# tsirigos/ibm-cbc-genomic-tools

Hardware: AMD Instinct MI355X
Metric: overlap-counted reads/sec, 100M reads x 1M ref intervals (higher is better)
Workload: dtype int32; 1 GPU; BASELINE config 3: 100000000 50bp reads in total, sorted by (chrom,start), x 1000000 ref intervals over 24 hg38 chromosomes, strand ignored (genomic_overlaps count -S -i); reads resident in HBM; total_reads=100000000, refs=1000000, reduce=none (one rank)

## Files before the change

### ibm-cbc-genomic-tools_amd/csrc/gtx_capi.hip

```cpp
#include <hip/hip_runtime.h>
#include <stdint.h>
#include <string.h>
#include <stdio.h>
#include <algorithm>
#include <functional>
#include <string>
#include <thread>
#include <vector>
#include "gtx.h"
#include "gtx_kernels.h"
#include "gtx_pairs.h"
#include "gtx_join.h"
#include "gtx_offset.h"
#include "gtx_signal.h"
#include "gtx_text.h"
#include "gtx_internal.h"

typedef unsigned long long u64;

static thread_local std::string g_create_error;

namespace {

template <class T, bool Pinned> class Buf {
 public:
  size_t cap = 0;
  Buf() = default;
  Buf(Buf &&o) noexcept { *this = std::move(o); }
  Buf &operator=(Buf &&o) noexcept { if (this != &o) { reset(); std::swap(cap, o.cap); std::swap(p_, o.p_); } return *this; }
  ~Buf() { reset(); }
  T *get() const { return p_; }
  explicit operator bool() const { return p_ != nullptr; }
  void reset() { if (p_) (void)(Pinned ? hipHostFree(p_) : hipFree(p_)); p_ = nullptr; cap = 0; }
  hipError_t alloc(size_t n)
  {
    reset();
    const hipError_t e = Pinned ? hipHostMalloc((void **)&p_, sizeof(T) * n) : hipMalloc((void **)&p_, sizeof(T) * n);
    if (e == hipSuccess) cap = n;
    return e;
  }
  hipError_t reserve(size_t need, size_t room) { if (need <= cap) return hipSuccess; hipError_t e = alloc(room); if (e == hipSuccess) cap = need; return e; }
  hipError_t reserve(size_t n) { return reserve(n, n); }
  hipError_t grow(size_t n) { return reserve(std::max<size_t>(n, 1)); }
 private:
  T *p_ = nullptr;
};
template <class T> using DevBuf = Buf<T, false>;
template <class T> using PinBuf = Buf<T, true>;

struct PlaceTable {
  DevBuf<int4> cls; DevBuf<int> rank; int shift = 0;
  gtx::PlaceTable view() const { gtx::PlaceTable t; t.cls = cls.get(); t.rank = rank.get(); t.shift = shift; return t; }
};

struct BucketTables {
  DevBuf<int> bkt; DevBuf<int4> clsCell; DevBuf<uint16_t> cellTab; int nB = 0, nCells = 0, cellShift = 0;
  gtx::BucketTable view() const
  {
    gtx::BucketTable t;
    const int *d = bkt.get();
    t.posHi = d; t.eLo = d + nB; t.eHi = d + 2 * nB; t.sLo = d + 3 * nB; t.sHi = d + 4 * nB; t.cls = d + 5 * nB; t.clsStart = d + 6 * nB; t.nB = nB;
    t.clsCell = clsCell.get(); t.cellTab = cellTab.get(); t.nCells = nCells; t.cellShift = cellShift;
    return t;
  }
};

struct BucketCuts { std::vector<int32_t> posHi, eLo, eHi, sLo, sHi, cls, clsStart; };

struct HistSet { DevBuf<u64> histA, histB, partA, partB, prefA, prefB; DevBuf<unsigned> flags; unsigned epoch = 0; unsigned long long draws = 0; };

struct CountIndex {
  DevBuf<int> sortedE, sortedS, segStart, posE, posS, classBase;
  DevBuf<int> sampE, sampS; int sampShift = 6, nSamp = 0;
  DevBuf<int> topE, topS;
  PlaceTable place;
  BucketTables bkt;
  HistSet hist;
  HistSet alt[GTXI_SHARE_STREAMS];
  DevBuf<gtx::DevInfo> info3; unsigned shareSeq = 0; unsigned shareTurn[GTXI_SHARE_STREAMS] = {}; const gtx::DevInfo *lastShareInfo = nullptr;
};

struct CoverIndex {
  DevBuf<u64> cov[12];
  DevBuf<int> sortedT, segT, topT, posTE, posTS, classBaseT;
  int64_t histLenT = 0;
  PlaceTable place;
  BucketTables bkt;
  bool ready = false;
};

struct RefExtras {
  DevBuf<int> refS, refE, refC;
  int nSpecial = 0; DevBuf<int4> specialRefs; DevBuf<int> specialIdx; DevBuf<u64> specialOut;
  struct PairIdx { DevBuf<int> mem; int n = 0; bool built = false; gtx::PairIndex ix = {}; } pairMulti, pairAll;
  DevBuf<int2> blkOf, blkIv; bool refBlocks = false;
  DevBuf<u64> pairAcc;
  DevBuf<long long> joinKey; std::vector<long long> h_joinKey; int joinMono = -1;
  DevBuf<int4> offRef; DevBuf<int8_t> refStrand;
  bool sigSet = false; double sigMin = 0, sigMax = 0; int64_t sigBins = 0; DevBuf<long long> sigRefLen;
};

struct Share { bool on = false; DevBuf<int> tiles; int nTiles = 0; DevBuf<int> regions; int64_t nRegions = 0, offset = 0; DevBuf<unsigned char> owned; };

struct TextSlot {
  DevBuf<char> text; DevBuf<unsigned> seg;
  DevBuf<unsigned> nl; DevBuf<int> tri, w;
  DevBuf<int> tri2; DevBuf<unsigned> blk; DevBuf<int> w2;
  DevBuf<int> flag; PinBuf<int> hostFlag; PinBuf<char> pin, seam; DevBuf<unsigned long long> sum;
  hipEvent_t evParsed = nullptr, evConsumed = nullptr, evCopied = nullptr; bool busy = false;
};

}

struct gtx_ctx {
  int device = 0;
  hipStream_t stream = nullptr;
  std::string err;

  int64_t nRefs = -1, nValid = 0;
  int nClasses = 0;
  std::vector<int32_t> h_seg;
  CountIndex ix;
// ... 10 lines not shown
  DevBuf<int4> side; DevBuf<unsigned> sideCount; int sideCap = 1 << 20; bool sideUsed = false;
  int specialMode = 0;
  bool tileSumsValid = true;
  int64_t histLen = 0;
  bool pairUsed = false;
  DevBuf<int4> pairQ; DevBuf<int2> pairQBlk, pairQIv;
  DevBuf<long long> joinOff, joinPart, joinCut; DevBuf<int> joinPairs, joinScratch; DevBuf<unsigned> joinBig;
  DevBuf<int> joinReads; DevBuf<int2> joinQBlk, joinQIv;
  DevBuf<gtx::JoinInfo> joinInfo;
  int64_t joinBuffer = 1ll << 26;
  DevBuf<long long> offInv, offOut, offCnt, offPart; DevBuf<int8_t> offQStrand;
  DevBuf<gtx::SignalInfo> sigInfo; DevBuf<unsigned long long> sigBins; DevBuf<long long> sigW;

  DevBuf<gtx::DevInfo> d_info;
  int infoCur = 0;
  PinBuf<gtx::DevInfo> h_info;

  hipStream_t copyStream = nullptr;
  DevBuf<char> stage[2]; DevBuf<int> stageW[2];
  PinBuf<char> pin[2];
  hipEvent_t evCopied[2] = {nullptr, nullptr}, evConsumed[2] = {nullptr, nullptr}; bool slotBusy[2] = {false, false};
  long long stageSeq = 0; bool directPending = false;
  int copyThreads = 8;
  DevBuf<u64> out;
  DevBuf<char> scratch;
  TextSlot text[2];
  long long textSeq = 0;
  DevBuf<int> textTable; DevBuf<char> textNames; unsigned textMask = 0, textBlobLen = 0;
  std::string textBlob;

  DevBuf<u64> micro;
  DevBuf<long long> scanTab;
  std::vector<long long> scanKey;
  int64_t scanTotalWindows = 0, scanTotalMicro = 0, scanTotalTiles = 0;
  BucketTables bktS; DevBuf<gtx::ScanPart> scanParts; int nScanParts = 0; std::vector<long long> scanBktKey; DevBuf<gtx::DevInfo> scanInfo;
  int64_t scanOwnBlocks = 0; DevBuf<long long> scanBounds; DevBuf<int> scanFlag;
  DevBuf<char> resReads; DevBuf<int> resWeights; hipEvent_t evRes[2] = {nullptr, nullptr};

  static constexpr int kProfSlots = 64;
  bool prof = false; long long profCalls = 0;
  int profEvery = 1; long long profSeq = 0; bool profThis = false;
  hipEvent_t evRing[kProfSlots][4] = {};
  hipEvent_t *ev = evRing[0];

  bool streamOpen = false; int64_t streamSeen = 0; int32_t streamLast[2] = {0, 0};
  struct ScanOpen { bool open = false, weighted = false; gtx::ScanArgs a; std::vector<int32_t> classLen; int64_t extent = 0; char prep = '1'; uint32_t flags = 0;
                    DevBuf<unsigned long long> labelSum; } scan;
  int64_t seamUnsorted = INT64_MAX;

  int64_t batchReads = 8ll << 20;
  int chunksPerWave = 0;
  int64_t waveSlots = 8192;
  int prefetch = 4;
};

#define HIPCHK(ctx, call) do { hipError_t e_ = (call); if (e_ != hipSuccess) { \
    (ctx)->err = std::string(#call) + ": " + hipGetErrorString(e_); return GTX_E_HIP; } } while (0)

static int fail(gtx_ctx *c, int code, const char *msg) { c->err = msg; return code; }

template <class T> static hipError_t upload(DevBuf<T> &b, const T *v, size_t n)
{
  hipError_t e = b.alloc(n);
  return e == hipSuccess ? hipMemcpy(b.get(), v, sizeof(T) * n, hipMemcpyHostToDevice) : e;
}

static int make_hist_set(gtx_ctx *c, HistSet &h, int64_t histLen)
{
  const size_t parts = (size_t)gtx::scan_tiles(histLen) + 2;
  HIPCHK(c, h.histA.alloc(histLen)); HIPCHK(c, h.histB.alloc(histLen)); HIPCHK(c, h.partA.alloc(parts)); HIPCHK(c, h.partB.alloc(parts));
  HIPCHK(c, h.prefA.alloc(histLen)); HIPCHK(c, h.prefB.alloc(histLen)); HIPCHK(c, h.flags.alloc(8 * parts));
  for (DevBuf<u64> *b : {&h.histA, &h.histB, &h.partA, &h.partB}) HIPCHK(c, hipMemset(b->get(), 0, sizeof(u64) * b->cap));
  HIPCHK(c, hipMemset(h.flags.get(), 0, sizeof(unsigned) * h.flags.cap));
  h.epoch = 0; h.draws = 0;
  return GTX_OK;
}

static int make_place_table(gtx_ctx *c, const std::vector<int32_t> &seg, const std::vector<int32_t> &arrA, const std::vector<int32_t> &arrB,
                            int nClasses, int64_t nv, PlaceTable &out)
{
  const int64_t budget = std::max<int64_t>(1024, nv / 8) + 2 * (int64_t)nClasses;
  auto cellsOf = [&](int cl, int sh) -> int64_t {
    if (seg[cl] == seg[cl + 1]) return 0;
    const int64_t top = std::max<int64_t>(0, std::max(arrA[seg[cl + 1] - 1], arrB[seg[cl + 1] - 1]));
    return (top >> sh) + 2;
  };
  int sh = 0;
  for (;; sh++) { int64_t t = 0; for (int cl = 0; cl < nClasses; cl++) t += cellsOf(cl, sh); if (t <= budget || sh >= 31) break; }
  std::vector<int4> pc(std::max(nClasses, 1));
  std::vector<int32_t> rank;
  for (int cl = 0; cl < nClasses; cl++) {
    const int64_t nc = cellsOf(cl, sh);
    pc[cl] = make_int4(seg[cl], seg[cl + 1], (int)(rank.size() / 2), (int)nc);
    int32_t ia = seg[cl], ib = seg[cl];
    for (int64_t k = 0; k < nc; k++) {
      const int64_t first = k << sh;
      if (k > 0) { while (ia < seg[cl + 1] && arrA[ia] < first) ia++; while (ib < seg[cl + 1] && arrB[ib] < first) ib++; }
      rank.push_back(ia); rank.push_back(ib);
    }
  }
  rank.push_back(0); rank.push_back(0);
  out.cls.reset(); out.rank.reset();
  HIPCHK(c, out.cls.alloc(pc.size()));
  HIPCHK(c, out.rank.alloc(rank.size()));
  HIPCHK(c, hipMemcpy(out.cls.get(), pc.data(), sizeof(int4) * pc.size(), hipMemcpyHostToDevice));
  HIPCHK(c, hipMemcpy(out.rank.get(), rank.data(), sizeof(int32_t) * rank.size(), hipMemcpyHostToDevice));
  out.shift = sh;
  return GTX_OK;
}

static int build_bucket_tables(gtx_ctx *c, BucketTables &t, BucketCuts &k, int nClasses, bool sync = false)
{
  t.nB = 0;
  const int nB = (int)k.posHi.size();
  if (nB == 0) return GTX_OK;
  const std::vector<int32_t> &posHi = k.posHi, &clsStart = k.clsStart;
  const int kCells = 4096;
  int sh = 0;
  auto cellsAt = [&](int shift) {
    int64_t total = 0;
    for (int cl = 0; cl < nClasses; cl++) {
      const int b0 = clsStart[cl], b1 = clsStart[cl + 1];
      total += b1 - b0 <= 1 ? b1 - b0 : ((((int64_t)posHi[b1 - 2] - posHi[b0]) >> shift) + 1);
    }
// ... 22 lines not shown
  if (sync) HIPCHK(c, hipStreamSynchronize(c->stream));
  HIPCHK(c, upload(t.bkt, all.data(), all.size()));
  HIPCHK(c, t.clsCell.alloc((size_t)nClasses + 1));
  HIPCHK(c, hipMemcpy(t.clsCell.get(), clsCell.data(), sizeof(int32_t) * clsCell.size(), hipMemcpyHostToDevice));
  HIPCHK(c, upload(t.cellTab, cellTab.data(), cellTab.size()));
  t.nB = nB;
  return GTX_OK;
}

extern "C" {

int gtx_version(void) { return 100; }

gtx_ctx *gtx_create(int device_id)
{
  int n = 0;
  hipError_t e = hipGetDeviceCount(&n);
  if (e != hipSuccess || n <= 0) {
    g_create_error = std::string("gtx_create: no usable HIP device (") + (e != hipSuccess ? hipGetErrorString(e) : "device count 0") +
                     "); this library has no CPU path";
    return nullptr;
  }
  if (device_id < 0 || device_id >= n) { g_create_error = "gtx_create: device id out of range"; return nullptr; }
  if ((e = hipSetDevice(device_id)) != hipSuccess) { g_create_error = std::string("hipSetDevice: ") + hipGetErrorString(e); return nullptr; }
  gtx_ctx *c = new gtx_ctx();
  c->device = device_id;
  { int cus = 0; if (hipDeviceGetAttribute(&cus, hipDeviceAttributeMultiprocessorCount, device_id) == hipSuccess && cus > 0) c->waveSlots = 32ll * cus; }
  if (c->d_info.alloc(2) != hipSuccess || c->h_info.alloc(2) != hipSuccess) {
    g_create_error = "gtx_create: allocation failed"; delete c; return nullptr;
  }
  gtx::DevInfo *hi = c->h_info.get();
  hi[1].first_unsorted = INT64_MAX; hi[1].n_no_class = 0; hi[1].n_degenerate = 0; hi[1].first_degenerate = INT64_MAX; hi[1].n_unplaced = 0; hi[1].fault = 0;
  hi[0] = hi[1];
  if (hipMemcpy(c->d_info.get(), &hi[1], sizeof(gtx::DevInfo), hipMemcpyHostToDevice) != hipSuccess ||
      hipMemcpy(c->d_info.get() + 1, &hi[1], sizeof(gtx::DevInfo), hipMemcpyHostToDevice) != hipSuccess) {
    g_create_error = "gtx_create: hipMemcpy failed"; delete c; return nullptr;
  }
  for (auto &slot : c->evRing) for (auto &ev : slot) if (hipEventCreate(&ev) != hipSuccess) { g_create_error = "gtx_create: hipEventCreate failed"; delete c; return nullptr; }
  if (hipStreamCreateWithFlags(&c->copyStream, hipStreamNonBlocking) != hipSuccess) { g_create_error = "gtx_create: hipStreamCreate failed"; delete c; return nullptr; }
  for (int k = 0; k < 2; k++)
    if (hipEventCreateWithFlags(&c->evCopied[k], hipEventDisableTiming) != hipSuccess || hipEventCreateWithFlags(&c->evConsumed[k], hipEventDisableTiming) != hipSuccess ||
        hipEventCreateWithFlags(&c->evRes[k], hipEventDisableTiming) != hipSuccess) {
      g_create_error = "gtx_create: hipEventCreate failed"; delete c; return nullptr;
    }
  { unsigned hc = std::thread::hardware_concurrency(); c->copyThreads = (int)std::max(1u, std::min(hc ? hc : 4u, 8u));
    if (const char *ct = getenv("GTX_COPY_THREADS")) if (atoi(ct) > 0) c->copyThreads = atoi(ct); }
  const char *cpw = getenv("GTX_CHUNKS_PER_WAVE");
  if (cpw && atoi(cpw) > 0) c->chunksPerWave = atoi(cpw);
  const char *br = getenv("GTX_BATCH_READS");
  if (br && atoll(br) > 0) c->batchReads = atoll(br);
  if (const char *bm = getenv("GTX_BUCKET_MIN_READS")) c->bucketMinReads = atoll(bm);
  const char *pf = getenv("GTX_READS_PER_LANE");
  if (pf && atoi(pf) > 0) c->prefetch = atoi(pf);
  return c;
}

void gtx_destroy(gtx_ctx *c)
{
  if (!c) return;
  (void)hipSetDevice(c->device);
  if (c->copyStream) (void)hipStreamSynchronize(c->copyStream);
  for (int k = 0; k < 2; k++)
    for (hipEvent_t e : {c->evCopied[k], c->evConsumed[k], c->evRes[k]}) if (e) (void)hipEventDestroy(e);
  if (c->copyStream) (void)hipStreamDestroy(c->copyStream);
  for (auto &t : c->text) for (hipEvent_t e : {t.evParsed, t.evConsumed, t.evCopied}) if (e) (void)hipEventDestroy(e);
  for (auto &slot : c->evRing) for (auto &ev : slot) if (ev) (void)hipEventDestroy(ev);
  delete c;
}

const char *gtx_last_error(const gtx_ctx *c) { return c ? c->err.c_str() : g_create_error.c_str(); }

int gtx_set_stream(gtx_ctx *c, void *s) { if (!c) return GTX_E_ARG; c->stream = (hipStream_t)s; return GTX_OK; }

int gtx_sync(gtx_ctx *c)
{
  if (!c) return GTX_E_ARG;
  HIPCHK(c, hipSetDevice(c->device));
  HIPCHK(c, hipStreamSynchronize(c->copyStream));
  HIPCHK(c, hipStreamSynchronize(c->stream));
  return GTX_OK;
}

void *gtx_host_alloc(gtx_ctx *c, size_t bytes)
{
  if (!c) return nullptr;
  void *p = nullptr;
  if (hipSetDevice(c->device) != hipSuccess || hipHostMalloc(&p, bytes ? bytes : 1, hipHostMallocPortable) != hipSuccess) { c->err = "gtx_host_alloc: hipHostMalloc failed"; (void)hipGetLastError(); return nullptr; }
  return p;
}

void gtx_host_free(gtx_ctx *c, void *p) { (void)c; if (p) (void)hipHostFree(p); }

int64_t gtx_n_refs(const gtx_ctx *c) { return c ? c->nRefs : -1; }

int gtx_set_refs(gtx_ctx *c, const int32_t *tri, int64_t m, int32_t nClasses) { return gtx_set_refs_ex(c, tri, m, nClasses, 0); }

int gtx_set_refs_ex(gtx_ctx *c, const int32_t *tri, int64_t m, int32_t nClasses, uint32_t flags)
{
  if (!c || m < 0 || (m > 0 && !tri)) return c ? fail(c, GTX_E_ARG, "gtx_set_refs: bad argument") : GTX_E_ARG;
  if (m >= (int64_t)INT32_MAX - 4096) return fail(c, GTX_E_ARG, "gtx_set_refs: too many reference regions");
  HIPCHK(c, hipSetDevice(c->device));
  int maxc = -1;
  for (int64_t k = 0; k < m; k++) {
    int32_t cl = tri[3 * k], s = tri[3 * k + 1], e = tri[3 * k + 2];
    if (cl < -1) return fail(c, GTX_E_RANGE, "gtx_set_refs: negative class id");
    if (s >= INT32_MAX - 1 || e >= INT32_MAX - 1) return fail(c, GTX_E_RANGE, "gtx_set_refs: coordinate >= 2^31-2");
// ... 227 lines not shown
static int pairs_batch(gtx_ctx *c, const void *d_reads, const void *d_weights, int64_t n)
{
  if (c->rx.pairMulti.n > 0) {
    HIPCHK(c, gtx::launch_pair_miss(d_reads, d_weights, n, c->rx.pairMulti.ix, gtx::RegionBlocks{c->rx.blkOf.get(), c->rx.blkIv.get()}, c->rx.pairAcc.get() + c->nRefs, c->stream));
    c->pairUsed = true;
  }
  return GTX_OK;
}

static int merge_batch(gtx_ctx *c, const void *d_reads, const void *d_weights, int64_t n)
{
  if (c->sideUsed && c->rx.nSpecial) HIPCHK(c, gtx::launch_special_refs(d_reads, d_weights, n, c->rx.specialRefs.get(), c->rx.nSpecial, c->specialMode, c->rx.specialOut.get(), c->stream));
  return GTX_OK;
}

static int merge_end(gtx_ctx *c, void *d_out)
{
  if (c->pairUsed) {
    c->pairUsed = false;
    HIPCHK(c, gtx::launch_pair_apply((u64 *)d_out, c->rx.pairAcc.get(), c->rx.pairAcc.get() + c->nRefs, c->nRefs, c->stream));
  }
  if (!c->sideUsed) return GTX_OK;
  c->sideUsed = false;
  HIPCHK(c, gtx::launch_side_reads(c->rx.refC.get(), c->rx.refS.get(), c->rx.refE.get(), c->nRefs, c->side.get(), c->sideCount.get(), c->sideCap, c->specialMode, (u64 *)d_out,
                                   c->d_info.get() + c->infoCur, c->stream));
  HIPCHK(c, gtx::launch_special_scatter(c->rx.specialIdx.get(), c->rx.specialOut.get(), c->rx.nSpecial, (u64 *)d_out, c->sideCount.get(), c->stream));
  return GTX_OK;
}

static int count_begin(gtx_ctx *c)
{
  if (c->histDirty) {
    HistSet &h = c->ix.hist;
    for (DevBuf<u64> *b : {&h.histA, &h.histB, &h.partA, &h.partB}) HIPCHK(c, hipMemsetAsync(b->get(), 0, sizeof(u64) * b->cap, c->stream));
  }
  if (c->histDirty || c->covDirty) HIPCHK(c, hipMemcpyAsync(c->d_info.get() + c->infoCur, &c->h_info.get()[1], sizeof(gtx::DevInfo), hipMemcpyHostToDevice, c->stream));
  if ((c->histDirty || c->covDirty) && c->sideCount.get()) {
    HIPCHK(c, hipMemsetAsync(c->sideCount.get(), 0, sizeof(unsigned), c->stream));
    if (c->rx.nSpecial) HIPCHK(c, hipMemsetAsync(c->rx.specialOut.get(), 0, sizeof(u64) * c->rx.nSpecial, c->stream));
  }
  if (c->histDirty && c->rx.pairAcc.get()) HIPCHK(c, hipMemsetAsync(c->rx.pairAcc.get(), 0, sizeof(u64) * 2 * (size_t)std::max<int64_t>(c->nRefs, 1), c->stream));
  c->sideUsed = false; c->pairUsed = false;
  c->histDirty = true; c->tileSumsValid = true;
  c->ix.lastShareInfo = nullptr;
  return GTX_OK;
}

static int finalize_set(gtx_ctx *c, HistSet &h, bool sumsValid, u64 *d_hits, gtx::DevInfo *info, gtx::DevInfo *infoNext, hipStream_t s,
                        const gtx::FinalizeShare *fs, bool hist32)
{
  if (++h.epoch == 0) { HIPCHK(c, hipMemsetAsync(h.flags.get(), 0, sizeof(unsigned) * h.flags.cap, s)); h.epoch = 1; h.draws = 0; }
  HIPCHK(c, gtx::launch_finalize(h.histA.get(), h.histB.get(), c->histLen, h.partA.get(), h.partB.get(), sumsValid, h.prefA.get(), h.prefB.get(),
                                 c->ix.posE.get(), c->ix.posS.get(), c->ix.classBase.get(), c->nRefs, d_hits, infoNext, s, fs, h.flags.get(), h.epoch, info,
                                 &h.draws, hist32));
  return GTX_OK;
}

static int count_end(gtx_ctx *c, void *d_hits, bool share = false, bool scatter = false, bool hist32 = false)
{
  const gtx::FinalizeShare fs = {c->share.tiles.get(), c->share.nTiles, c->share.regions.get(), c->share.nRegions, scatter};
  int rc = finalize_set(c, c->ix.hist, c->tileSumsValid, (u64 *)d_hits, c->d_info.get() + c->infoCur, c->d_info.get() + (c->infoCur ^ 1), c->stream,
                        share ? &fs : nullptr, hist32);
  if (rc) return rc;
  rc = merge_end(c, d_hits); if (rc) return rc;
  c->histDirty = false;
  c->infoCur ^= 1;
  return GTX_OK;
}

int gtx_count_device(gtx_ctx *c, const void *d_reads, const void *d_weights, int64_t n, uint32_t flags, void *d_hits)
{
  if (!c) return GTX_E_ARG;
  if (c->nRefs < 0) return fail(c, GTX_E_STATE, "gtx_count_device: gtx_set_refs has not been called");
  if (n < 0 || (n > 0 && !d_reads) || (c->nRefs > 0 && !d_hits)) return fail(c, GTX_E_ARG, "gtx_count_device: bad argument");
  HIPCHK(c, hipSetDevice(c->device));
  int rc = count_begin(c); if (rc) return rc;
  c->profThis = c->prof && (c->profEvery <= 1 || (c->profSeq++ % c->profEvery) == 0);
  if (c->profThis) { c->ev = c->evRing[c->profCalls % gtx_ctx::kProfSlots]; HIPCHK(c, hipEventRecord(c->ev[1], c->stream)); }
  rc = merge_prepare(c, flags, 0); if (rc) return rc;
  const bool streaming = (flags & (GTX_READS_SORTED | GTX_CHECK_SORTED)) != 0;
  if (!streaming) c->tileSumsValid = false;
  bool h32 = false;
  if (streaming) {
    const gtx::CountArgs a = count_args(c, c->ix.hist, flags, n, 0, COUNT_ANY, d_weights == nullptr);
    h32 = a.hist32 != 0 && n > 0;
    HIPCHK(c, gtx::launch_count(d_reads, d_weights, n, a, true, c->stream));
  }
  else { rc = launch_unsorted(c, d_reads, d_weights, n, count_args(c, c->ix.hist, flags, n)); if (rc) return rc; }
  rc = merge_batch(c, d_reads, d_weights, n); if (rc) return rc;
  rc = pairs_batch(c, d_reads, d_weights, n); if (rc) return rc;
  if (c->profThis) HIPCHK(c, hipEventRecord(c->ev[2], c->stream));
  rc = count_end(c, d_hits, false, false, h32); if (rc) return rc;
  if (c->profThis) { if (c->profEvery <= 1) HIPCHK(c, hipEventRecord(c->ev[3], c->stream)); c->profCalls++; }
  return GTX_OK;
}

static void info_out(const gtx::DevInfo &d, gtx_count_info *o, int64_t base)
{
  o->first_unsorted = d.first_unsorted == INT64_MAX ? -1 : d.first_unsorted + base;
  o->n_no_class = d.n_no_class; o->n_degenerate = d.n_degenerate;
  o->first_degenerate = d.first_degenerate == INT64_MAX ? -1 : d.first_degenerate + base;
  o->n_unplaced = d.n_unplaced;
}

static int fault_check(gtx_ctx *c, const gtx::DevInfo &d)
{
  return d.fault ? fail(c, GTX_E_HIP, "the finalize step gave up waiting for a tile sum (finalize_scan_chained_kernel): the result of this call is void; GTX_CHAINED_SCAN=0 takes the two-launch finalize") : GTX_OK;
// ... 1606 lines not shown
```

### ibm-cbc-genomic-tools_amd/csrc/gtx_kernels.h

```cpp
#pragma once
#include <hip/hip_runtime.h>
#include <stdint.h>
#include <mutex>

namespace gtx {

struct PerDevice {
  std::mutex m; unsigned long long done = 0;
  template <class F> hipError_t once(F fn)
  {
    int dev = 0;
    hipError_t e = hipGetDevice(&dev);
    if (e != hipSuccess) return e;
    std::lock_guard<std::mutex> lk(m);
    if (dev >= 0 && dev < 64 && ((done >> dev) & 1)) return hipSuccess;
    e = fn();
    if (e == hipSuccess && dev >= 0 && dev < 64) done |= 1ull << dev;
    return e;
  }
};

struct DevInfo {
  long long first_unsorted;
  long long n_no_class;
// ... 93 lines not shown
  const int *cls;
  const int *clsStart;
  int nB;
  const int4 *clsCell;
  const unsigned short *cellTab;
  int nCells, cellShift;
};
struct BucketWork {
  void *tmpReads; int *tmpWeights;
  unsigned arenaPairs;
  unsigned *dir;
  unsigned *list;
  unsigned *chunkCount;
  unsigned *rowOff;
  unsigned *arenaUsed;
};
struct BucketPlan { int per, line; unsigned blocks; size_t arenaPairs, pairs, chunks, matrix; };
BucketPlan bucket_plan(long long n, int nClasses, int nB, int nCells, bool weighted);
bool bucket_tables_fit(int nClasses, int nB, int nCells);
int bucket_e_size();
int bucket_s_size();
int bucket_t_size();
hipError_t launch_count_bucketed(const void *reads, const void *weights, long long n, const CountArgs &a, const BucketTable &t,
                                 const BucketWork &w, const BucketPlan &p, hipStream_t st);
hipError_t launch_cover_bucketed(const void *reads, const void *weights, long long n, const CountArgs &a, const CoverArgs &cv, const BucketTable &t,
                                 const BucketWork &w, const BucketPlan &p, hipStream_t st);
struct ScanPart { int bucket, first, count, pad; };
int scan_part_bins(bool weighted);
hipError_t launch_scan_bucketed(const void *reads, const void *weights, long long n, const CountArgs &a, const ScanArgs &sc, const BucketTable &t,
                                const BucketWork &w, const BucketPlan &p, const ScanPart *parts, int nParts, hipStream_t st,
                                unsigned long long *out = nullptr);
int scan_fused_max_comb();
hipError_t launch_tile_sums(unsigned long long *histA, unsigned long long *histB, long long histLen, unsigned long long *tileA, unsigned long long *tileB, hipStream_t st);

hipError_t launch_special_refs(const void *reads, const void *weights, long long n, const int4 *refs, int nSpecial, int mode,
                               unsigned long long *out, hipStream_t st);
hipError_t launch_side_reads(const int *refC, const int *refS, const int *refE, long long m, const int4 *side, const unsigned *sideCount,
                             int sideCap, int mode, unsigned long long *hits, DevInfo *info, hipStream_t st);
hipError_t launch_special_scatter(const int *specialIdx, unsigned long long *specialOut, int nSpecial, unsigned long long *hits,
                                  unsigned *sideCount, hipStream_t st);

SpanSchedule span_schedule(long long nChunks, int cpw, int r, long long slots);
int search_sample_shift(long long nValid);
int scan_tiles(long long len);

hipError_t launch_count(const void *reads, const void *weights, long long n, const CountArgs &a, bool sortedHint, hipStream_t st);
struct FinalizeShare { const int *tileList; int nTiles; const int *regionList; long long nRegions; bool scatter; };
hipError_t launch_finalize(unsigned long long *histA, unsigned long long *histB, long long histLen,
                           unsigned long long *tileA, unsigned long long *tileB, bool tileSumsValid,
                           unsigned long long *prefA, unsigned long long *prefB,
                           const int *posE, const int *posS, const int *classBase, long long m,
                           unsigned long long *hits, DevInfo *nextInfo, hipStream_t st, const FinalizeShare *share = nullptr,
                           unsigned *chainFlags = nullptr, unsigned epoch = 0, DevInfo *info = nullptr, unsigned long long *chainDraws = nullptr,
                           bool hist32 = false);
hipError_t launch_coverage(const void *reads, const void *weights, long long n, const CoverArgs &a, hipStream_t st);
hipError_t launch_coverage_finalize(const CoverArgs &a, long long histLen, const CoverGather &g, long long m,
                                    unsigned long long *cov, DevInfo *nextInfo, hipStream_t st);
hipError_t launch_scan_zero(void *micro, long long bytes, const int *runIf, hipStream_t st);
hipError_t launch_scan_hist(const void *reads, const void *weights, long long n, const ScanArgs &a, hipStream_t st, const int *runIf = nullptr);
int scan_window_tile();
hipError_t launch_scan_windows(const void *micro, bool micro64, const ScanArgs &a, long long totalTiles,
                               unsigned long long *out, hipStream_t st, const int *runIf = nullptr);

struct ScanOwn {
  const long long *blkOff;
  int tile;
  long long totalBlocks;
  long long *bounds;
  int *flag;
};
int scan_own_tile(long long nReads, long long totalMicro, int comb);
hipError_t launch_scan_own(const void *reads, const void *weights, long long n, const ScanArgs &a, const ScanOwn &o,
                           unsigned long long *out, hipStream_t st);

}
```

### ibm-cbc-genomic-tools_amd/csrc/gtx_kernels.hip

```cpp
#include <hip/hip_runtime.h>
#include <stdint.h>
#include <stdlib.h>
#include <string.h>
#include <stdio.h>
#include <type_traits>
#include <vector>
#include <algorithm>
#include "gtx_kernels.h"

namespace gtx {

typedef unsigned long long u64;
typedef long long i64;

static constexpr int kHi = 0x7fffffff;
static constexpr int kLo = (int)0x80000000;
static constexpr int kSlots = 63;
static constexpr int kTileShift = 10;
static constexpr int kTile = 1 << kTileShift;
static constexpr int kSearchLdsBytes = 128 * 1024;

__device__ __forceinline__ int rfl(int v) { return __builtin_amdgcn_readfirstlane(v); }
__device__ __forceinline__ int rdlane(int v, int l) { return __builtin_amdgcn_readlane(v, l); }

// ... 1266 lines not shown

template <class T>
__global__ __launch_bounds__(256) void tile_sums_kernel(const T *__restrict__ ha, const T *__restrict__ hb, i64 len,
                                                        u64 *__restrict__ pa, u64 *__restrict__ pb, const int *__restrict__ tileList)
{
  __shared__ u64 lds[4];
  const T *__restrict__ h = blockIdx.y ? hb : ha;
  const int tileIdx = tileList ? tileList[blockIdx.x] : (int)blockIdx.x;
  const i64 i0 = (i64)tileIdx * kTile + (i64)threadIdx.x * 4;
  u64 s = 0;
  if (i0 + 4 <= len) { u64 v[4]; load4<T>(h + i0, v); s = v[0] + v[1] + v[2] + v[3]; }
  else for (int k = 0; k < 4; k++) if (i0 + k < len) s += h[i0 + k];
  s = block_sum(s, lds);
  if (threadIdx.x == 0) (blockIdx.y ? pb : pa)[tileIdx] = s;
}

template <class T>
__global__ __launch_bounds__(256) void finalize_scan_kernel(T *__restrict__ ha, T *__restrict__ hb, i64 len,
                                                            const u64 *__restrict__ ta, const u64 *__restrict__ tb,
                                                            T *__restrict__ pa, T *__restrict__ pb, const int *__restrict__ tileList)
{
  __shared__ u64 lds[4];
  __shared__ u64 wsum[4];
  T *__restrict__ h = blockIdx.y ? hb : ha;
  const u64 *__restrict__ ts = blockIdx.y ? tb : ta;
  T *__restrict__ p = blockIdx.y ? pb : pa;
  const int lane = threadIdx.x & 63, wv = threadIdx.x >> 6;
  const int tile = tileList ? tileList[blockIdx.x] : (int)blockIdx.x;
  const i64 i0 = (i64)tile * kTile + (i64)threadIdx.x * 4;
  const bool full = i0 + 4 <= len;
  u64 v[4];
  if (full) load4<T>(h + i0, v);
  else {
#pragma unroll
    for (int k = 0; k < 4; k++) v[k] = i0 + k < len ? (u64)h[i0 + k] : 0;
  }
  u64 o = 0;
  for (int t = threadIdx.x; t < tile; t += 256) o += ts[t];
  o = block_sum(o, lds);
  v[1] += v[0]; v[2] += v[1]; v[3] += v[2];
  const u64 x = wave_scan_add64(v[3]);
  if (lane == 63) wsum[wv] = x;
  __syncthreads();
  o += x - v[3];
  for (int k = 0; k < wv; k++) o += wsum[k];
  if (full) { store4<T>(p + i0, v[0] + o, v[1] + o, v[2] + o, v[3] + o); store4<T>(h + i0, 0, 0, 0, 0); }
  else {
#pragma unroll
    for (int k = 0; k < 4; k++)
      if (i0 + k < len) { p[i0 + k] = (T)(v[k] + o); h[i0 + k] = 0; }
  }
}

static constexpr unsigned kChainSpinMax = 1u << 22;
static constexpr int kChainMaxTiles = 512;
template <class T>
__global__ __launch_bounds__(256) void finalize_scan_chained_kernel(T *__restrict__ ha, T *__restrict__ hb, i64 len,
                                                                    u64 *fa, u64 *fb, u64 *ctlA, u64 *ctlB, u64 base, unsigned epoch, int nRun,
                                                                    T *__restrict__ pa, T *__restrict__ pb, const int *__restrict__ tileList,
                                                                    DevInfo *info)
{
  __shared__ u64 lds[4];
  __shared__ u64 wsum[4];
  __shared__ u64 tk;
  const bool second = blockIdx.y != 0;
  if (threadIdx.x == 0) tk = atomicAdd(second ? ctlB : ctlA, 1ull) - base;
  __syncthreads();
  if (tk >= (u64)nRun) { if (threadIdx.x == 0) atomicAdd((u64 *)&info->fault, 1ull); return; }
  T *__restrict__ h = second ? hb : ha;
  u64 *fl = second ? fb : fa;
  T *__restrict__ p = second ? pb : pa;
  const int lane = threadIdx.x & 63, wv = threadIdx.x >> 6;
  const int pos = (int)tk, tile = tileList ? tileList[pos] : pos;
  const i64 i0 = (i64)tile * kTile + (i64)threadIdx.x * 4;
  const bool full = i0 + 4 <= len;
  u64 v[4];
  if (full) load4<T>(h + i0, v);
  else {
#pragma unroll
    for (int k = 0; k < 4; k++) v[k] = i0 + k < len ? (u64)h[i0 + k] : 0;
  }
  v[1] += v[0]; v[2] += v[1]; v[3] += v[2];
  const u64 x = wave_scan_add64(v[3]);
  if (lane == 63) wsum[wv] = x;
  __syncthreads();
  if (threadIdx.x < 2) {
    const u64 s = wsum[0] + wsum[1] + wsum[2] + wsum[3];
    __hip_atomic_store(fl + 2 * pos + threadIdx.x, ((u64)epoch << 32) | (threadIdx.x ? s >> 32 : s & 0xffffffffull), __ATOMIC_RELAXED, __HIP_MEMORY_SCOPE_AGENT);
  }
  u64 o = 0;
  bool gaveUp = false;
  for (int t = threadIdx.x; t < pos; t += 256) {
    u64 lo, hi; unsigned spins = 0;
    while (((lo = __hip_atomic_load(fl + 2 * t, __ATOMIC_RELAXED, __HIP_MEMORY_SCOPE_AGENT)) >> 32) != epoch && ++spins < kChainSpinMax) __builtin_amdgcn_s_sleep(1);
    while (((hi = __hip_atomic_load(fl + 2 * t + 1, __ATOMIC_RELAXED, __HIP_MEMORY_SCOPE_AGENT)) >> 32) != epoch && ++spins < kChainSpinMax) __builtin_amdgcn_s_sleep(1);
    if (spins >= kChainSpinMax) { gaveUp = true; break; }
    o += (lo & 0xffffffffull) | (hi << 32);
  }
  if (gaveUp) atomicAdd((u64 *)&info->fault, 1ull);
  o = block_sum(o, lds);
  o += x - v[3];
  for (int k = 0; k < wv; k++) o += wsum[k];
  if (full) { store4<T>(p + i0, v[0] + o, v[1] + o, v[2] + o, v[3] + o); store4<T>(h + i0, 0, 0, 0, 0); }
  else {
#pragma unroll
    for (int k = 0; k < 4; k++)
      if (i0 + k < len) { p[i0 + k] = (T)(v[k] + o); h[i0 + k] = 0; }
  }
}

template <class T>
__global__ __launch_bounds__(256) void gather_hits_kernel(const T *__restrict__ pa, const T *__restrict__ pb,
                                                          const int *__restrict__ posE, const int *__restrict__ posS,
                                                          const int *__restrict__ classBase, i64 m, u64 *__restrict__ hits,
                                                          u64 *__restrict__ ta, u64 *__restrict__ tb, int nTiles, DevInfo *nextInfo,
                                                          const int *__restrict__ regionList, int scatter)
{
  i64 k = (i64)blockIdx.x * blockDim.x + threadIdx.x;
  if (k < nTiles) { ta[k] = 0; tb[k] = 0; }
  if (k == 0) { nextInfo->first_unsorted = INT64_MAX; nextInfo->n_no_class = 0; nextInfo->n_degenerate = 0; nextInfo->first_degenerate = INT64_MAX; nextInfo->n_unplaced = 0; nextInfo->fault = 0; }
  if (k >= m) return;
  i64 outIdx = k;
  if (regionList) { k = regionList[k]; if (scatter) outIdx = k; }
  int pe = posE[k];
  u64 h = 0;
  if (pe >= 0) {
    int cb = classBase[k];
    T ba = cb >= 0 ? pa[cb] : 0, bb = cb >= 0 ? pb[cb] : 0;
    h = (u64)(T)((T)(pa[pe] - ba) - (T)(pb[posS[k]] - bb));
  }
  hits[outIdx] = h;
}

__global__ __launch_bounds__(256) void gather_coverage_kernel(CoverGather g, i64 m, u64 *__restrict__ cov, int nTiles, DevInfo *nextInfo)
{
  i64 k = (i64)blockIdx.x * blockDim.x + threadIdx.x;
  if (k < nTiles) {
#pragma unroll
    for (int q = 0; q < 4; q++) g.part[q][k] = 0;
  }
  if (k == 0) { nextInfo->first_unsorted = INT64_MAX; nextInfo->n_no_class = 0; nextInfo->n_degenerate = 0; nextInfo->first_degenerate = INT64_MAX; nextInfo->n_unplaced = 0; nextInfo->fault = 0; }
  if (k >= m) return;
  const int pe = g.posTE[k];
  u64 c = 0;
  if (pe >= 0 && g.refE[k] >= g.refS[k]) {
    const int ps = g.posTS[k], cb = g.classBaseT[k];
    u64 v[8];
#pragma unroll
    for (int q = 0; q < 4; q++) { const u64 *p = g.pref[q]; const u64 b = cb >= 0 ? p[cb] : 0; v[q] = p[pe] - b; v[4 + q] = p[ps] - b; }
    const u64 E = (u64)(i64)g.refE[k], S = (u64)(i64)g.refS[k];
    c = v[3] - v[7] + E * (v[0] - v[2]) - v[1] + v[5] - S * (v[4] - v[6]) + v[0] - v[6];
  }
  cov[k] = c;
}

__device__ __forceinline__ void scan_slot(const Tri &t, bool in_range, const ScanArgs &a, int &cls, int &mw, int clsU = -1, i64 nmU = 0)
{
  cls = -1; mw = -1;
  if (in_range && (clsU >= 0 || (unsigned)t.c < (unsigned)a.nClasses) && (a.sortedRule || (t.s <= t.e && t.e > 0))) {
    i64 pos = a.center ? (i64)t.s + ((i64)t.e - t.s) / 2 : (i64)t.s;
    if (a.sortedRule && pos < 1) pos = 1;
    if (pos >= 1) {
      const unsigned x = (unsigned)(pos - 1), d = (unsigned)a.winStep;
      unsigned q = d == 1 ? x : __umulhi(x, a.winStepInv);
      unsigned r = x - q * d;
      if (r >= d) { q++; r -= d; }
      if (r >= d) q++;
      if ((i64)q < (clsU >= 0 ? nmU : a.nMicro[t.c])) { cls = t.c; mw = (int)q; }
    }
  }
}

static constexpr int kScanTile = 1024;

template <bool WEIGHTED>
struct ScanTile { typedef typename std::conditional<WEIGHTED, u64, unsigned>::type ct; ct *lds; int cls, base; bool used; };

template <bool WEIGHTED>
__device__ __forceinline__ void scan_tile_flush(ScanTile<WEIGHTED> &T, const ScanArgs &a, int lane)
{
  typedef typename ScanTile<WEIGHTED>::ct ct;
  if (!T.used) return;
  ct *dst = (ct *)a.micro + a.microOff[T.cls] + T.base;
  for (int k = 0; k < kScanTile; k += 64) {
// ... 188 lines not shown
    s.wave0[k] = (int)wave; s.chunk0[k] = (int)chunk; s.cpw[k] = tail[i].cpw; wave += w; chunk += w * tail[i].cpw; ++k;
  }
  s.nSeg = k; s.nWaves = wave;
  return s;
}

hipError_t launch_count(const void *reads, const void *weights, i64 n, const CountArgs &a, bool sortedHint, hipStream_t st)
{
  if (n <= 0) return hipSuccess;
  if (sortedHint) {
    const i64 waves = a.sched.nWaves;
    static const int wpb = getenv("GTX_WAVES_PER_BLOCK") ? std::min(4, std::max(1, atoi(getenv("GTX_WAVES_PER_BLOCK")))) : 4;
    const unsigned grid = (unsigned)((waves + wpb - 1) / wpb);
    const unsigned bs = 64u * wpb;
    static const bool wfast = !(getenv("GTX_WEIGHTED_FAST") && atoi(getenv("GTX_WEIGHTED_FAST")) == 0);
    if (weights && wfast) count_walk_kernel_weighted<<<grid, bs, 0, st>>>((const Tri *)reads, (const int *)weights, n, a);
    else if (weights) count_walk_kernel<true, 2><<<grid, bs, 0, st>>>((const Tri *)reads, (const int *)weights, n, a);
    else if (a.prefetch <= 1) count_walk_kernel<false, 1><<<grid, bs, 0, st>>>((const Tri *)reads, (const int *)weights, n, a);
    else if (a.prefetch == 2) count_walk_kernel<false, 2><<<grid, bs, 0, st>>>((const Tri *)reads, (const int *)weights, n, a);
    else if (a.prefetch == 3) count_walk_kernel<false, 3><<<grid, bs, 0, st>>>((const Tri *)reads, (const int *)weights, n, a);
    else if (a.flip && a.hist32) count_walk_kernel_flip_h32<<<grid, bs, 0, st>>>((const Tri *)reads, (const int *)weights, n, a);
    else if (a.flip) count_walk_kernel_flip<<<grid, bs, 0, st>>>((const Tri *)reads, (const int *)weights, n, a);
    else if (a.hist32) count_walk_kernel_h32<<<grid, bs, 0, st>>>((const Tri *)reads, (const int *)weights, n, a);
    else if (getenv("GTX_PF") && atoi(getenv("GTX_PF"))) count_walk_kernel_pf<<<grid, bs, 0, st>>>((const Tri *)reads, (const int *)weights, n, a);
    else count_walk_kernel<false, 4><<<grid, bs, 0, st>>>((const Tri *)reads, (const int *)weights, n, a);
  } else {
    static PerDevice attr;
    {
      hipError_t e = attr.once([] {
        hipError_t e2 = hipFuncSetAttribute((const void *)count_search_kernel<true>, hipFuncAttributeMaxDynamicSharedMemorySize, kSearchLdsBytes);
        if (e2 == hipSuccess) e2 = hipFuncSetAttribute((const void *)count_search_kernel<false>, hipFuncAttributeMaxDynamicSharedMemorySize, kSearchLdsBytes);
        return e2;
      });
      if (e != hipSuccess) return e;
    }
    i64 blocks = (n + 1023) / 1024; if (blocks > 512) blocks = 512;
    const size_t lds = sizeof(int) * 2 * (size_t)a.nSamp;
    if (weights) count_search_kernel<true><<<(unsigned)blocks, 1024, lds, st>>>((const Tri *)reads, (const int *)weights, n, a);
    else count_search_kernel<false><<<(unsigned)blocks, 1024, lds, st>>>((const Tri *)reads, (const int *)weights, n, a);
  }
  return hipGetLastError();
}

hipError_t launch_tile_sums(u64 *histA, u64 *histB, i64 histLen, u64 *tileA, u64 *tileB, hipStream_t st)
{
  const int nb = scan_tiles(histLen);
  if (nb > 0) tile_sums_kernel<u64><<<dim3(nb, 2), 256, 0, st>>>(histA, histB, histLen, tileA, tileB, nullptr);
  return hipGetLastError();
}

template <class T>
static hipError_t launch_finalize_t(T *histA, T *histB, i64 histLen, u64 *tileA, u64 *tileB, bool tileSumsValid, T *prefA, T *prefB,
                                    const int *posE, const int *posS, const int *classBase, i64 m, u64 *hits, DevInfo *nextInfo, hipStream_t st,
                                    const FinalizeShare *share, unsigned *chainFlags, unsigned epoch, DevInfo *info, unsigned long long *chainDraws)
{
  const int nb = scan_tiles(histLen);
  const int nbRun = share ? share->nTiles : nb;
  const int *tl = share ? share->tileList : nullptr;
  static const bool chained = !(getenv("GTX_CHAINED_SCAN") && atoi(getenv("GTX_CHAINED_SCAN")) == 0);
  if (nbRun > 0) {
    static const int chainMax = getenv("GTX_CHAIN_MAX_TILES") ? atoi(getenv("GTX_CHAIN_MAX_TILES")) : kChainMaxTiles;
    if (!tileSumsValid && chainFlags && chained && info && chainDraws && nbRun <= chainMax) {
      finalize_scan_chained_kernel<T><<<dim3(nbRun, 2), 256, 0, st>>>(histA, histB, histLen, (u64 *)chainFlags, (u64 *)chainFlags + 2 * (nb + 2), (u64 *)chainFlags + 2 * nb,
                                                                      (u64 *)chainFlags + 2 * (nb + 2) + 2 * nb, *chainDraws, epoch, nbRun, prefA, prefB, tl, info);
      *chainDraws += (unsigned long long)nbRun;
    }
    else {
      if (!tileSumsValid) tile_sums_kernel<T><<<dim3(nbRun, 2), 256, 0, st>>>(histA, histB, histLen, tileA, tileB, tl);
      finalize_scan_kernel<T><<<dim3(nbRun, 2), 256, 0, st>>>(histA, histB, histLen, tileA, tileB, prefA, prefB, tl);
    }
  }
  const i64 mm = share ? share->nRegions : m;
  const i64 work = (mm > nb ? mm : nb) > 0 ? (mm > nb ? mm : nb) : 1;
  gather_hits_kernel<T><<<(unsigned)((work + 255) / 256), 256, 0, st>>>(prefA, prefB, posE, posS, classBase, mm, hits, tileA, tileB, nb, nextInfo,
                                                                        share ? share->regionList : nullptr, share && share->scatter ? 1 : 0);
  return hipGetLastError();
}

hipError_t launch_finalize(u64 *histA, u64 *histB, i64 histLen, u64 *tileA, u64 *tileB, bool tileSumsValid, u64 *prefA, u64 *prefB,
                           const int *posE, const int *posS, const int *classBase, i64 m, u64 *hits, DevInfo *nextInfo, hipStream_t st,
                           const FinalizeShare *share, unsigned *chainFlags, unsigned epoch, DevInfo *info, unsigned long long *chainDraws, bool hist32)
{
  if (hist32) return launch_finalize_t<unsigned>((unsigned *)histA, (unsigned *)histB, histLen, tileA, tileB, tileSumsValid, (unsigned *)prefA, (unsigned *)prefB,
                                                 posE, posS, classBase, m, hits, nextInfo, st, share, chainFlags, epoch, info, chainDraws);
  return launch_finalize_t<u64>(histA, histB, histLen, tileA, tileB, tileSumsValid, prefA, prefB, posE, posS, classBase, m, hits, nextInfo, st, share, chainFlags, epoch,
                                info, chainDraws);
}

hipError_t launch_coverage(const void *reads, const void *weights, i64 n, const CoverArgs &a, hipStream_t st)
{
  if (n <= 0) return hipSuccess;
  const i64 waves = a.sched.nWaves;
  const unsigned grid = (unsigned)((waves + 3) / 4);
  if (weights) coverage_walk_kernel_weighted<<<grid, 256, 0, st>>>((const Tri *)reads, (const int *)weights, n, a);
  else coverage_walk_kernel<false><<<grid, 256, 0, st>>>((const Tri *)reads, (const int *)weights, n, a);
  return hipGetLastError();
}

hipError_t launch_coverage_finalize(const CoverArgs &a, i64 histLen, const CoverGather &g, i64 m, u64 *cov, DevInfo *nextInfo, hipStream_t st)
{
  const int nb = scan_tiles(histLen);
  for (int q = 0; q < 4 && nb > 0; q += 2)
    finalize_scan_kernel<u64><<<dim3(nb, 2), 256, 0, st>>>(a.hist[q], a.hist[q + 1], histLen, a.part[q], a.part[q + 1], g.pref[q], g.pref[q + 1], nullptr);
  const i64 work = (m > nb ? m : nb) > 0 ? (m > nb ? m : nb) : 1;
  gather_coverage_kernel<<<(unsigned)((work + 255) / 256), 256, 0, st>>>(g, m, cov, nb, nextInfo);
  return hipGetLastError();
}

__global__ __launch_bounds__(256) void scan_zero_kernel(uint4 *__restrict__ p, i64 n16, const int *__restrict__ runIf)
{
  if (runIf && *runIf == 0) return;
  for (i64 i = (i64)blockIdx.x * blockDim.x + threadIdx.x; i < n16; i += (i64)gridDim.x * blockDim.x) p[i] = make_uint4(0, 0, 0, 0);
}

hipError_t launch_scan_zero(void *micro, i64 bytes, const int *runIf, hipStream_t st)
{
  const i64 n16 = (bytes + 15) / 16;
  if (n16 <= 0) return hipSuccess;
  i64 blocks = (n16 + 255) / 256; if (blocks > 4096) blocks = 4096;
  scan_zero_kernel<<<(unsigned)blocks, 256, 0, st>>>((uint4 *)micro, n16, runIf);
  return hipGetLastError();
}

hipError_t launch_scan_hist(const void *reads, const void *weights, i64 n, const ScanArgs &a, hipStream_t st, const int *runIf)
{
  if (n <= 0) return hipSuccess;
  static const int perCuEnv = getenv("GTX_SCAN_BLOCKS_PER_CU") ? atoi(getenv("GTX_SCAN_BLOCKS_PER_CU")) : 0;
  const int perCu = perCuEnv > 0 ? perCuEnv : (weights ? 16 : 32);
  i64 blocks = (n + 4095) / 4096; if (blocks > 256 * (i64)perCu) blocks = 256 * (i64)perCu;
  if (weights) scan_hist_kernel<true><<<(unsigned)blocks, 256, 0, st>>>((const Tri *)reads, (const int *)weights, n, a, runIf);
  else scan_hist_kernel<false><<<(unsigned)blocks, 256, 0, st>>>((const Tri *)reads, (const int *)weights, n, a, runIf);
  return hipGetLastError();
}

int scan_window_tile() { return kWinTile; }

hipError_t launch_scan_windows(const void *micro, bool micro64, const ScanArgs &a, i64 totalTiles, u64 *out, hipStream_t st, const int *runIf)
{
  if (totalTiles <= 0) return hipSuccess;
// ... 7 lines not shown
```

Baseline: 466.1 billion reads/s.

## Add tile-local finalize scan with tile-offset fixup folded into gather

Adds a finalize path that scans each histogram tile independently and writes per-tile totals. A large-block gather kernel then scans those totals in shared memory and adds the tile offset while computing the hits. This avoids the separate tile-sums pass that precedes a global scan when the chained scan is not used. It applies only when the tile count is at most 4096 and no tile list is given; the chained path still takes precedence for small tile counts. The cost is a 1024-thread gather kernel with a large shared-memory footprint and a cap of 512 blocks, and it adds a new buffer per histogram set.

```diff
diff --git a/ibm-cbc-genomic-tools_amd/csrc/gtx_capi.hip b/ibm-cbc-genomic-tools_amd/csrc/gtx_capi.hip
--- a/ibm-cbc-genomic-tools_amd/csrc/gtx_capi.hip
+++ b/ibm-cbc-genomic-tools_amd/csrc/gtx_capi.hip
@@ -67,7 +67,7 @@
 
 struct BucketCuts { std::vector<int32_t> posHi, eLo, eHi, sLo, sHi, cls, clsStart; };
 
-struct HistSet { DevBuf<u64> histA, histB, partA, partB, prefA, prefB; DevBuf<unsigned> flags; unsigned epoch = 0; unsigned long long draws = 0; };
+struct HistSet { DevBuf<u64> histA, histB, partA, partB, prefA, prefB, tot; DevBuf<unsigned> flags; unsigned epoch = 0; unsigned long long draws = 0; };
 
 struct CountIndex {
   DevBuf<int> sortedE, sortedS, segStart, posE, posS, classBase;
@@ -184,6 +184,7 @@
   int chunksPerWave = 0;
   int64_t waveSlots = 8192;
   int prefetch = 4;
+  bool finalizeLocal = true;
 };
 
 #define HIPCHK(ctx, call) do { hipError_t e_ = (call); if (e_ != hipSuccess) { \
@@ -201,7 +202,7 @@
 {
   const size_t parts = (size_t)gtx::scan_tiles(histLen) + 2;
   HIPCHK(c, h.histA.alloc(histLen)); HIPCHK(c, h.histB.alloc(histLen)); HIPCHK(c, h.partA.alloc(parts)); HIPCHK(c, h.partB.alloc(parts));
-  HIPCHK(c, h.prefA.alloc(histLen)); HIPCHK(c, h.prefB.alloc(histLen)); HIPCHK(c, h.flags.alloc(8 * parts));
+  HIPCHK(c, h.prefA.alloc(histLen)); HIPCHK(c, h.prefB.alloc(histLen)); HIPCHK(c, h.flags.alloc(8 * parts)); HIPCHK(c, h.tot.alloc(2 * parts));
   for (DevBuf<u64> *b : {&h.histA, &h.histB, &h.partA, &h.partB}) HIPCHK(c, hipMemset(b->get(), 0, sizeof(u64) * b->cap));
   HIPCHK(c, hipMemset(h.flags.get(), 0, sizeof(unsigned) * h.flags.cap));
   h.epoch = 0; h.draws = 0;
@@ -330,6 +331,7 @@
   if (const char *bm = getenv("GTX_BUCKET_MIN_READS")) c->bucketMinReads = atoll(bm);
   const char *pf = getenv("GTX_READS_PER_LANE");
   if (pf && atoi(pf) > 0) c->prefetch = atoi(pf);
+  if (const char *fl = getenv("GTX_FINALIZE_LOCAL")) c->finalizeLocal = atoi(fl) != 0;
   return c;
 }
 
@@ -663,7 +665,7 @@
   if (++h.epoch == 0) { HIPCHK(c, hipMemsetAsync(h.flags.get(), 0, sizeof(unsigned) * h.flags.cap, s)); h.epoch = 1; h.draws = 0; }
   HIPCHK(c, gtx::launch_finalize(h.histA.get(), h.histB.get(), c->histLen, h.partA.get(), h.partB.get(), sumsValid, h.prefA.get(), h.prefB.get(),
                                  c->ix.posE.get(), c->ix.posS.get(), c->ix.classBase.get(), c->nRefs, d_hits, infoNext, s, fs, h.flags.get(), h.epoch, info,
-                                 &h.draws, hist32));
+                                 &h.draws, hist32, c->finalizeLocal ? h.tot.get() : nullptr));
   return GTX_OK;
 }
 
diff --git a/ibm-cbc-genomic-tools_amd/csrc/gtx_kernels.h b/ibm-cbc-genomic-tools_amd/csrc/gtx_kernels.h
--- a/ibm-cbc-genomic-tools_amd/csrc/gtx_kernels.h
+++ b/ibm-cbc-genomic-tools_amd/csrc/gtx_kernels.h
@@ -169,7 +169,7 @@
                            const int *posE, const int *posS, const int *classBase, long long m,
                            unsigned long long *hits, DevInfo *nextInfo, hipStream_t st, const FinalizeShare *share = nullptr,
                            unsigned *chainFlags = nullptr, unsigned epoch = 0, DevInfo *info = nullptr, unsigned long long *chainDraws = nullptr,
-                           bool hist32 = false);
+                           bool hist32 = false, unsigned long long *tileTotals = nullptr);
 hipError_t launch_coverage(const void *reads, const void *weights, long long n, const CoverArgs &a, hipStream_t st);
 hipError_t launch_coverage_finalize(const CoverArgs &a, long long histLen, const CoverGather &g, long long m,
                                     unsigned long long *cov, DevInfo *nextInfo, hipStream_t st);
diff --git a/ibm-cbc-genomic-tools_amd/csrc/gtx_kernels.hip b/ibm-cbc-genomic-tools_amd/csrc/gtx_kernels.hip
--- a/ibm-cbc-genomic-tools_amd/csrc/gtx_kernels.hip
+++ b/ibm-cbc-genomic-tools_amd/csrc/gtx_kernels.hip
@@ -1342,6 +1342,38 @@
   }
 }
 
+template <class T>
+__global__ __launch_bounds__(256) void finalize_local_kernel(T *__restrict__ ha, T *__restrict__ hb, i64 len, T *__restrict__ pa, T *__restrict__ pb,
+                                                             u64 *__restrict__ tota, u64 *__restrict__ totb)
+{
+  __shared__ u64 wsum[4];
+  T *__restrict__ h = blockIdx.y ? hb : ha;
+  T *__restrict__ p = blockIdx.y ? pb : pa;
+  const int lane = threadIdx.x & 63, wv = threadIdx.x >> 6;
+  const int tile = (int)blockIdx.x;
+  const i64 i0 = (i64)tile * kTile + (i64)threadIdx.x * 4;
+  const bool full = i0 + 4 <= len;
+  u64 v[4];
+  if (full) load4<T>(h + i0, v);
+  else {
+#pragma unroll
+    for (int k = 0; k < 4; k++) v[k] = i0 + k < len ? (u64)h[i0 + k] : 0;
+  }
+  v[1] += v[0]; v[2] += v[1]; v[3] += v[2];
+  const u64 x = wave_scan_add64(v[3]);
+  if (lane == 63) wsum[wv] = x;
+  __syncthreads();
+  u64 o = x - v[3];
+  for (int k = 0; k < wv; k++) o += wsum[k];
+  if (full) { store4<T>(p + i0, v[0] + o, v[1] + o, v[2] + o, v[3] + o); store4<T>(h + i0, 0, 0, 0, 0); }
+  else {
+#pragma unroll
+    for (int k = 0; k < 4; k++)
+      if (i0 + k < len) { p[i0 + k] = (T)(v[k] + o); h[i0 + k] = 0; }
+  }
+  if (threadIdx.x == 255) (blockIdx.y ? totb : tota)[tile] = v[3] + o;
+}
+
 static constexpr unsigned kChainSpinMax = 1u << 22;
 static constexpr int kChainMaxTiles = 512;
 template <class T>
@@ -1420,6 +1452,77 @@
     h = (u64)(T)((T)(pa[pe] - ba) - (T)(pb[posS[k]] - bb));
   }
   hits[outIdx] = h;
+}
+
+static constexpr int kFinalizeLocalMaxTiles = 4096;
+static constexpr int kGatherLocalBlocks = 512;
+template <class T>
+__global__ __launch_bounds__(1024) void gather_hits_local_kernel(const T *__restrict__ pa, const T *__restrict__ pb,
+                                                                 const u64 *__restrict__ tota, const u64 *__restrict__ totb, int nTiles,
+                                                                 const int *__restrict__ posE, const int *__restrict__ posS,
+                                                                 const int *__restrict__ classBase, i64 m, u64 *__restrict__ hits, DevInfo *nextInfo,
+                                                                 const int *__restrict__ regionList, int scatter, u64 *__restrict__ ta, u64 *__restrict__ tb)
+{
+  __shared__ T off[2][kFinalizeLocalMaxTiles];
+  __shared__ u64 wsum[16];
+  const int lane = threadIdx.x & 63, wv = threadIdx.x >> 6, half = threadIdx.x >> 9;
+  if (blockIdx.x == 0 && threadIdx.x == 0) { nextInfo->first_unsorted = INT64_MAX; nextInfo->n_no_class = 0; nextInfo->n_degenerate = 0; nextInfo->first_degenerate = INT64_MAX; nextInfo->n_unplaced = 0; nextInfo->fault = 0; }
+  const u64 *__restrict__ tot = half ? totb : tota;
+  const int per = (nTiles + 511) >> 9, t0 = (int)(threadIdx.x & 511) * per;
+  u64 tv[8], s = 0;
+#pragma unroll
+  for (int q = 0; q < 8; q++) {
+    tv[q] = 0;
+    if (q < per) { const u64 x = tot[t0 + q < nTiles ? t0 + q : nTiles - 1]; tv[q] = t0 + q < nTiles ? x : 0; }
+    s += tv[q];
+  }
+  const i64 stride = (i64)gridDim.x * blockDim.x;
+  i64 j = (i64)blockIdx.x * blockDim.x + threadIdx.x;
+  for (i64 t = j; t < nTiles; t += stride) { ta[t] = 0; tb[t] = 0; }
+  if (m <= 0) return;
+  i64 out[2]; int pe[2], ps[2], cb[2]; T a[2], b[2], ba[2], bb[2];
+  auto fetch = [&]() {
+    i64 k[2];
+#pragma unroll
+    for (int r = 0; r < 2; r++) { const i64 jr = j + r * stride; out[r] = jr < m ? jr : -1; k[r] = jr < m ? jr : 0; }
+    if (regionList) {
+#pragma unroll
+      for (int r = 0; r < 2; r++) { k[r] = regionList[k[r]]; if (scatter && out[r] >= 0) out[r] = k[r]; }
+    }
+#pragma unroll
+    for (int r = 0; r < 2; r++) { pe[r] = posE[k[r]]; ps[r] = posS[k[r]]; cb[r] = classBase[k[r]]; }
+#pragma unroll
+    for (int r = 0; r < 2; r++) {
+      const int e = pe[r] > 0 ? pe[r] : 0, st = pe[r] >= 0 && ps[r] > 0 ? ps[r] : 0, c = cb[r] > 0 ? cb[r] : 0;
+      a[r] = pa[e]; b[r] = pb[st]; ba[r] = pa[c]; bb[r] = pb[c];
+    }
+  };
+  fetch();
+  const u64 x = wave_scan_add64(s);
+  if (lane == 63) wsum[wv] = x;
+  __syncthreads();
+  u64 o = x - s;
+  for (int k = half * 8; k < wv; k++) o += wsum[k];
+#pragma unroll
+  for (int q = 0; q < 8; q++)
+    if (q < per && t0 + q < nTiles) { off[half][t0 + q] = (T)o; o += tv[q]; }
+  __syncthreads();
+  while (j < m) {
+#pragma unroll
+    for (int r = 0; r < 2; r++) {
+      u64 h = 0;
+      if (pe[r] >= 0) {
+        const int st = ps[r] > 0 ? ps[r] : 0;
+        const T va = a[r] + off[0][pe[r] >> kTileShift], vb = b[r] + off[1][st >> kTileShift];
+        T vba = 0, vbb = 0;
+        if (cb[r] >= 0) { vba = ba[r] + off[0][cb[r] >> kTileShift]; vbb = bb[r] + off[1][cb[r] >> kTileShift]; }
+        h = (u64)(T)((T)(va - vba) - (T)(vb - vbb));
+      }
+      if (out[r] >= 0) hits[out[r]] = h;
+    }
+    j += 2 * stride;
+    if (j < m) fetch();
+  }
 }
 
 __global__ __launch_bounds__(256) void gather_coverage_kernel(CoverGather g, i64 m, u64 *__restrict__ cov, int nTiles, DevInfo *nextInfo)
@@ -1714,39 +1817,51 @@
 template <class T>
 static hipError_t launch_finalize_t(T *histA, T *histB, i64 histLen, u64 *tileA, u64 *tileB, bool tileSumsValid, T *prefA, T *prefB,
                                     const int *posE, const int *posS, const int *classBase, i64 m, u64 *hits, DevInfo *nextInfo, hipStream_t st,
-                                    const FinalizeShare *share, unsigned *chainFlags, unsigned epoch, DevInfo *info, unsigned long long *chainDraws)
+                                    const FinalizeShare *share, unsigned *chainFlags, unsigned epoch, DevInfo *info, unsigned long long *chainDraws,
+                                    u64 *tileTotals)
 {
   const int nb = scan_tiles(histLen);
   const int nbRun = share ? share->nTiles : nb;
   const int *tl = share ? share->tileList : nullptr;
+  const i64 mm = share ? share->nRegions : m;
+  const int *rl = share ? share->regionList : nullptr;
+  const int scatter = share && share->scatter ? 1 : 0;
   static const bool chained = !(getenv("GTX_CHAINED_SCAN") && atoi(getenv("GTX_CHAINED_SCAN")) == 0);
   if (nbRun > 0) {
     static const int chainMax = getenv("GTX_CHAIN_MAX_TILES") ? atoi(getenv("GTX_CHAIN_MAX_TILES")) : kChainMaxTiles;
     if (!tileSumsValid && chainFlags && chained && info && chainDraws && nbRun <= chainMax) {
       finalize_scan_chained_kernel<T><<<dim3(nbRun, 2), 256, 0, st>>>(histA, histB, histLen, (u64 *)chainFlags, (u64 *)chainFlags + 2 * (nb + 2), (u64 *)chainFlags + 2 * nb,
                                                                       (u64 *)chainFlags + 2 * (nb + 2) + 2 * nb, *chainDraws, epoch, nbRun, prefA, prefB, tl, info);
+      const hipError_t e = hipGetLastError();
+      if (e != hipSuccess) return e;
       *chainDraws += (unsigned long long)nbRun;
+    }
+    else if (!tileSumsValid && tileTotals && !tl && nb <= kFinalizeLocalMaxTiles) {
+      finalize_local_kernel<T><<<dim3(nb, 2), 256, 0, st>>>(histA, histB, histLen, prefA, prefB, tileTotals, tileTotals + nb);
+      const i64 blocks = (mm + 2047) / 2048;
+      gather_hits_local_kernel<T><<<(unsigned)(blocks < 1 ? 1 : blocks > kGatherLocalBlocks ? kGatherLocalBlocks : blocks), 1024, 0, st>>>(
+          prefA, prefB, tileTotals, tileTotals + nb, nb, posE, posS, classBase, mm, hits, nextInfo, rl, scatter, tileA, tileB);
+      return hipGetLastError();
     }
     else {
       if (!tileSumsValid) tile_sums_kernel<T><<<dim3(nbRun, 2), 256, 0, st>>>(histA, histB, histLen, tileA, tileB, tl);
       finalize_scan_kernel<T><<<dim3(nbRun, 2), 256, 0, st>>>(histA, histB, histLen, tileA, tileB, prefA, prefB, tl);
     }
   }
-  const i64 mm = share ? share->nRegions : m;
   const i64 work = (mm > nb ? mm : nb) > 0 ? (mm > nb ? mm : nb) : 1;
-  gather_hits_kernel<T><<<(unsigned)((work + 255) / 256), 256, 0, st>>>(prefA, prefB, posE, posS, classBase, mm, hits, tileA, tileB, nb, nextInfo,
-                                                                        share ? share->regionList : nullptr, share && share->scatter ? 1 : 0);
+  gather_hits_kernel<T><<<(unsigned)((work + 255) / 256), 256, 0, st>>>(prefA, prefB, posE, posS, classBase, mm, hits, tileA, tileB, nb, nextInfo, rl, scatter);
   return hipGetLastError();
 }
 
 hipError_t launch_finalize(u64 *histA, u64 *histB, i64 histLen, u64 *tileA, u64 *tileB, bool tileSumsValid, u64 *prefA, u64 *prefB,
                            const int *posE, const int *posS, const int *classBase, i64 m, u64 *hits, DevInfo *nextInfo, hipStream_t st,
-                           const FinalizeShare *share, unsigned *chainFlags, unsigned epoch, DevInfo *info, unsigned long long *chainDraws, bool hist32)
+                           const FinalizeShare *share, unsigned *chainFlags, unsigned epoch, DevInfo *info, unsigned long long *chainDraws, bool hist32,
+                           u64 *tileTotals)
 {
   if (hist32) return launch_finalize_t<unsigned>((unsigned *)histA, (unsigned *)histB, histLen, tileA, tileB, tileSumsValid, (unsigned *)prefA, (unsigned *)prefB,
-                                                 posE, posS, classBase, m, hits, nextInfo, st, share, chainFlags, epoch, info, chainDraws);
+                                                 posE, posS, classBase, m, hits, nextInfo, st, share, chainFlags, epoch, info, chainDraws, tileTotals);
   return launch_finalize_t<u64>(histA, histB, histLen, tileA, tileB, tileSumsValid, prefA, prefB, posE, posS, classBase, m, hits, nextInfo, st, share, chainFlags, epoch,
-                                info, chainDraws);
+                                info, chainDraws, tileTotals);
 }
 
 hipError_t launch_coverage(const void *reads, const void *weights, i64 n, const CoverArgs &a, hipStream_t st)
```

Measured after the change: 474.3 billion reads/s (median of 6 runs). +1.8%, better.
